# 10XGenomics/supernova

Measured on AMD Instinct MI355X. Metric: Gk-mers/s through count+graph at k=48, 1.2B×150bp; bit-exact counts, higher is better.
Workload: dtype u64

## Files before the change

supernova_amd/csrc/snk_graph.h:

```cpp
#pragma once
#include "snk_ctx.h"
#include "snk_kernels.h"

struct snk_graph_out {
    uint8_t* ctx;
    uint32_t* counts;
    unsigned long long* spectrum;
    uint32_t spectrum_bins;
    uint64_t n_unitigs;
    uint64_t total_bases;
    uint64_t* unitig_off;
    uint8_t* unitig_bases;
    uint32_t* unitig_group;
    uint32_t n_circles;
    uint32_t rank_rounds;
    uint64_t n_boundary;
    uint64_t n_fragments;
};

int snk_graph_sort(snk_ctx* ctx, hipStream_t st, uint32_t K, uint64_t n, snk_u128* keys_in, uint64_t* vals_in,
                   snk_u128* keys_out, uint64_t* vals_out, char* err, size_t errcap);
int snk_graph_build(snk_ctx* ctx, hipStream_t st, uint32_t K, const snk_u128* keys, const uint64_t* vals, uint64_t n,
                    uint32_t do_prune, bool want_unitigs, snk_graph_out* out, char* err, size_t errcap);

// ... 39 lines not shown
int snk_join_rank(snk_ctx* ctx, hipStream_t st, uint64_t F, const uint32_t* nk, uint32_t* flink, const uint2** rk_out, uint8_t** circ_out,
                  uint32_t* n_circles, uint32_t* rounds, char* err, size_t errcap, uint8_t* circ_given = nullptr);
int snk_join_place(snk_ctx* ctx, hipStream_t st, const uint2* rk, const uint32_t* nk, const uint8_t* circ, uint64_t f0, uint64_t Fl,
                   snk_placement* pl, char* err, size_t errcap, uint64_t rk_f0 = 0);
struct snk_prank {
    uint64_t ns, m, k0, k1, n_rec;
    const uint32_t* w;
    uint32_t* link;
    unsigned long long* wrec;
    uint32_t* spl_state;
    uint4* w1_share;
    uint4* rec;
};
int snk_prank_begin(snk_ctx* ctx, hipStream_t st, uint64_t F, const uint32_t* nk, uint32_t* link, uint32_t rank, uint32_t world, snk_prank* P, char* err,
                    size_t errcap);
int snk_prank_walk(snk_ctx* ctx, hipStream_t st, snk_prank* P, const uint4* w1_all, uint32_t* circles, uint32_t* rounds, char* err, size_t errcap,
                   uint8_t* circ = nullptr , uint32_t* n_cut = nullptr);
int snk_prank_route(snk_ctx* ctx, hipStream_t st, snk_prank* P, const unsigned long long* d_frag_off, uint32_t world,
                    unsigned long long* d_cursor , void* d_out, char* err, size_t errcap);
int snk_prank_apply(snk_ctx* ctx, hipStream_t st, const void* d_rec, uint64_t n, unsigned long long state_base, uint64_t n_local_states,
                    const uint2** rk_out, char* err, size_t errcap);
int snk_join_emit(snk_ctx* ctx, hipStream_t st, uint32_t K, uint64_t F, const uint32_t* nk, const uint32_t* gfid, const uint32_t* pl_pid,
                  const unsigned long long* pl_koff, const unsigned long long* pl_N, const uint8_t* pl_circ, uint32_t pid_base, uint64_t n_pid,
                  const uint64_t* boff, const uint8_t* fbases, const uint32_t* fgroup, snk_join_out* out, char* err, size_t errcap);
int snk_dist_answer(snk_ctx* ctx, hipStream_t st, snk_dist_graph* g, const void* d_queries, uint64_t nq, void* d_ans, char* err,
                    size_t errcap);
int snk_dist_apply(snk_ctx* ctx, hipStream_t st, snk_dist_graph* g, const void* d_qbuf, const void* d_ans, uint64_t nq,
                   const unsigned long long* d_qoff, char* err, size_t errcap);
int snk_dist_join(snk_ctx* ctx, hipStream_t st, uint32_t K, uint64_t F, const uint32_t* nk, const unsigned long long* hl_self,
                  const unsigned long long* hl_nb, const uint64_t* boff, const uint8_t* fbases, uint64_t total_fbases,
                  snk_join_out* out, char* err, size_t errcap, const uint32_t* fgroup = nullptr, const uint32_t* sfrag = nullptr,
                  uint64_t n_states = 0);
int snk_dist_links_query(snk_ctx* ctx, hipStream_t st, const snk_frag_out* fr, const unsigned long long* d_node_off, uint32_t world,
                         unsigned long long my_end_base, unsigned long long* d_cursor, void* d_qbuf, char* err, size_t errcap);
int snk_dist_links_answer(snk_ctx* ctx, hipStream_t st, const snk_frag_out* fr, const void* d_queries, uint64_t nq, unsigned long long my_state_base,
                          uint64_t n_local_states, unsigned long long my_end_base, void* d_ans, char* err, size_t errcap);
int snk_dist_links_apply_regions(snk_ctx* ctx, hipStream_t st, const snk_frag_out* fr, const void* d_qbuf, const void* d_ans, uint32_t world, uint64_t cap,
                                 const unsigned long long* counts, uint32_t** flink_out, char* err, size_t errcap);

struct snk_table;
struct snk_bl_state {
    const snk_table* tab;
    uint32_t K, rank, world, NB_total, NBl, do_prune, force_dist;
    uint4* desc;
    uint32_t nchunks, nbig;
    uint32_t* biglist;
    uint8_t *ctx, *pend, *premote;
    uint32_t *counts, *nbr, *rq;
    uint32_t* rq_idx;
    uint16_t* rq_meta;
    unsigned long long* index;
    uint64_t index_mask, n_boundary;
    unsigned long long *qcount, *qcursor;
    unsigned long long* spec;
    uint32_t want_spec, spec_over;
// ... 11 lines not shown
```

supernova_amd/csrc/snk_graph.hip:

```cpp
#include <string.h>
#include <cstring>
#include <rocprim/rocprim.hpp>

#include "snk_ctx.h"
#include "snk_common.h"
#include "snk_kernels.h"
#include "snk_graph.h"
#include "snk_stages.h"

namespace {

constexpr uint32_t NONE = 0xFFFFFFFFu;
constexpr int TB = 256;

__device__ __forceinline__ snk_kmer load_key(const snk_u128* keys, uint64_t i) {
    const uint64_t* p = reinterpret_cast<const uint64_t*>(keys + i);
    snk_kmer k;
    k.lo = p[0];
    k.hi = p[1];
    return k;
}

__global__ void __launch_bounds__(TB) index_build_kernel(const snk_u128* __restrict__ keys, uint64_t n,
                                                         unsigned long long* __restrict__ tab, uint64_t mask) {
// ... 1066 lines not shown
__device__ __forceinline__ uint32_t ld_u32_any(const uint8_t* p) { return reinterpret_cast<const u32_any*>(p)->v; }
__device__ __forceinline__ void st_u32_any(uint8_t* p, uint32_t v) { reinterpret_cast<u32_any*>(p)->v = v; }
__device__ __forceinline__ void copy16(uint8_t* dst, const uint8_t* src, bool rev) {
    if (!rev) {
        const uint32_t a = ld_u32_any(src), b = ld_u32_any(src + 4), c = ld_u32_any(src + 8), d = ld_u32_any(src + 12);
        st_u32_any(dst, a); st_u32_any(dst + 4, b); st_u32_any(dst + 8, c); st_u32_any(dst + 12, d);
    } else {
        const uint32_t a = ld_u32_any(src - 4), b = ld_u32_any(src - 8), c = ld_u32_any(src - 12), d = ld_u32_any(src - 16);
        st_u32_any(dst, __builtin_bswap32(a) ^ 0x03030303u); st_u32_any(dst + 4, __builtin_bswap32(b) ^ 0x03030303u);
        st_u32_any(dst + 8, __builtin_bswap32(c) ^ 0x03030303u); st_u32_any(dst + 12, __builtin_bswap32(d) ^ 0x03030303u);
    }
}
constexpr uint32_t JCH = 4096;
__global__ void __launch_bounds__(TB) jchunks_kernel(const uint64_t* __restrict__ boff, uint64_t F, uint32_t* __restrict__ nch) {
    uint64_t f = (uint64_t)blockIdx.x * TB + threadIdx.x;
    if (f >= F) return;
    nch[f] = (uint32_t)((boff[f + 1] - boff[f] + JCH - 1) / JCH);
}
__global__ void __launch_bounds__(TB) jchunk_owner_kernel(const uint32_t* __restrict__ choff, uint64_t F, uint32_t* __restrict__ owner) {
    uint64_t f = (uint64_t)blockIdx.x * TB + threadIdx.x;
    if (f >= F) return;
    if (choff[f + 1] > choff[f]) owner[choff[f]] = (uint32_t)f;
}
__global__ void __launch_bounds__(256) jemit_kernel(uint64_t F, const uint64_t* __restrict__ boff, const uint8_t* __restrict__ fbases,
                                                    const uint32_t* __restrict__ pl_pid, const unsigned long long* __restrict__ pl_koff,
                                                    const uint32_t* __restrict__ nk, const uint64_t* __restrict__ poff, uint32_t pid_base,
                                                    uint32_t K, uint8_t* __restrict__ prov) {
    for (uint64_t f = (uint64_t)blockIdx.x * 32 + (threadIdx.x >> 3); f < F; f += (uint64_t)gridDim.x * 32) {
    const uint32_t sub = threadIdx.x & 7u;
    const unsigned long long ko = pl_koff[f];
    const bool rc = (ko & PL_RC) != 0;
    const uint32_t skip = (ko & ~PL_RC) == 0 ? 0u : K - 1;
    const uint32_t len = nk[f] + K - 1 - skip;
    const uint8_t* src = fbases + boff[f] + (rc ? 0u : skip);
    uint8_t* dst = prov + poff[pl_pid[f] - pid_base] + (ko & ~PL_RC) + skip;
    uint32_t head = (4u - (uint32_t)((uintptr_t)dst & 3u)) & 3u;
    if (head > len) head = len;
    if (sub < head) dst[sub] = rc ? (uint8_t)(src[len - 1 - sub] ^ 3u) : src[sub];
    const uint32_t ndw = (len - head) >> 2;
    for (uint32_t j = sub; j < ndw; j += 8) {
        const uint32_t o = head + 4 * j;
        const uint32_t v = rc ? (__builtin_bswap32(ld_u32_any(src + len - 4 - o)) ^ 0x03030303u) : ld_u32_any(src + o);
        *reinterpret_cast<uint32_t*>(dst + o) = v;
    }
    const uint32_t t0 = head + 4 * ndw;
    if (sub < len - t0) { const uint32_t q = t0 + sub; dst[q] = rc ? (uint8_t)(src[len - 1 - q] ^ 3u) : src[q]; }
    }
}
__global__ void __launch_bounds__(TB) jform_kernel(const uint64_t* __restrict__ uoff, uint64_t U, const uint8_t* __restrict__ prov,
                                                   uint8_t* __restrict__ urev) {
    uint64_t u = (uint64_t)blockIdx.x * TB + threadIdx.x;
    if (u >= U) return;
    const uint8_t* b = prov + uoff[u];
    uint64_t len = uoff[u + 1] - uoff[u];
    uint8_t rev = 0;
    if (len & 1) rev = (b[len / 2] & 2) ? 1 : 0;
    else {
        for (uint64_t i = 0, j = len; i < j; ++i) {
            uint8_t f = b[i], r = (uint8_t)(b[--j] ^ 3);
            if (f < r) break;
            if (r < f) { rev = 1; break; }
        }
    }
    urev[u] = rev;
}
__global__ void __launch_bounds__(TB) jfinal_kernel(const uint64_t* __restrict__ uoff, const uint32_t* __restrict__ uowner_of_chunk,
                                                    const uint32_t* __restrict__ uchoff, const uint8_t* __restrict__ urev,
                                                    const uint8_t* __restrict__ prov, uint8_t* __restrict__ out) {
    const uint32_t item = blockIdx.x;
// ... 144 lines not shown
        void* tmp;
        if ((rc = snk_ctx_alloc(ctx, tb, &tmp, err, errcap))) return rc;
        SNK_HIP_TRY(rocprim::inclusive_scan(tmp, tb, owner, owner, (size_t)total, rocprim::maximum<uint32_t>(), st));
    }
    *choff_out = choff;
    *owner_out = owner;
    *total_out = total;
    return SNK_OK;
}

int snk_dist_answer(snk_ctx* ctx, hipStream_t st, snk_dist_graph* g, const void* d_queries, uint64_t nq, void* d_ans, char* err,
                    size_t errcap) {
    SNK_HIP_TRY(snk_launch(answer_kernel, snk_blocks(nq, TB), TB, 0, st, (const unsigned long long*)d_queries, nq, g->keys, g->index, g->index_mask, (uint32_t*)d_ans));
    return SNK_OK;
}
int snk_dist_apply(snk_ctx* ctx, hipStream_t st, snk_dist_graph* g, const void* d_qbuf, const void* d_ans, uint64_t nq,
                   const unsigned long long* d_qoff, char* err, size_t errcap) {
    SNK_HIP_TRY(snk_launch(apply_answers_kernel, snk_blocks(nq, TB), TB, 0, st, (const unsigned long long*)d_qbuf, (const uint32_t*)d_ans, nq, d_qoff, g->world, g->do_prune, reinterpret_cast<uint32_t*>(g->ctx), g->rq_idx, g->rq_meta));
    return SNK_OK;
}

int snk_dist_join(snk_ctx* ctx, hipStream_t st, uint32_t K, uint64_t F, const uint32_t* nk, const unsigned long long* hl_self,
                  const unsigned long long* hl_nb, const uint64_t* boff, const uint8_t* fbases, uint64_t total_fbases,
                  snk_join_out* out, char* err, size_t errcap, const uint32_t* fgroup, const uint32_t* sfrag, uint64_t n_states) {
    memset(out, 0, sizeof *out);
    if (F == 0) return snk_join_emit(ctx, st, K, 0, nullptr, nullptr, nullptr, nullptr, nullptr, nullptr, 0, 0, nullptr, nullptr, nullptr, out, err, errcap);
    if (F >= (1ull << 31)) return snk_fail(SNK_E_UNSUPPORTED, err, errcap, "more than 2^31 fragments at the join (%llu)", (unsigned long long)F);
    const uint64_t ne = 2 * F;
    uint32_t* flink;
    G_ALLOC(flink, uint32_t, ne);
    if (sfrag) {
        SNK_HIP_TRY(snk_launch(jmatch_direct_kernel, snk_blocks(ne, TB), TB, 0, st, hl_self, hl_nb, ne, sfrag, n_states, flink));
    } else {
        uint64_t tg = 1024;
        while (tg < 2 * ne) tg <<= 1;
        unsigned long long* hk;
        uint32_t* hv;
        G_ALLOC(hk, unsigned long long, tg);
        G_ALLOC(hv, uint32_t, tg);
        SNK_HIP_TRY(hipMemsetAsync(hk, 0, tg * 8, st));
        SNK_HIP_TRY(snk_launch(jhash_build_kernel, snk_blocks(ne, TB), TB, 0, st, hl_self, ne, hk, hv, tg - 1));
        SNK_HIP_TRY(snk_launch(jmatch_kernel, snk_blocks(ne, TB), TB, 0, st, hl_self, hl_nb, ne, hk, hv, tg - 1, flink));
    }
    uint8_t* circ;
    G_ALLOC(circ, uint8_t, ne + 1);
    SNK_HIP_TRY(hipMemsetAsync(circ, 0, ne + 1, st));
    const uint2* rk;
    int rc = rank_lists(ctx, st, flink, F, nk, circ, &rk, &out->n_circles, &out->rank_rounds, err, errcap);
    if (rc) return rc;
    snk_placement pl;
    if ((rc = snk_join_place(ctx, st, rk, nk, circ, 0, F, &pl, err, errcap))) return rc;
    const uint32_t nc = out->n_circles, rr = out->rank_rounds;
    if ((rc = snk_join_emit(ctx, st, K, F, nk, nullptr, pl.pid, pl.koff, pl.N, pl.circ, 0, ne, boff, fbases, fgroup, out, err, errcap))) return rc;
    out->n_circles = nc;
    out->rank_rounds = rr;
    return SNK_OK;
}

int snk_join_rank(snk_ctx* ctx, hipStream_t st, uint64_t F, const uint32_t* nk, uint32_t* flink, const uint2** rk_out, uint8_t** circ_out,
                  uint32_t* n_circles, uint32_t* rounds, char* err, size_t errcap, uint8_t* circ_given) {
    if (F >= (1ull << 31)) return snk_fail(SNK_E_UNSUPPORTED, err, errcap, "more than 2^31 fragments at the join (%llu)", (unsigned long long)F);
    uint8_t* circ = circ_given;
    if (!circ) {
        G_ALLOC(circ, uint8_t, 2 * F + 1);
        SNK_HIP_TRY(hipMemsetAsync(circ, 0, 2 * F + 1, st));
    }
    *circ_out = circ;
    *n_circles = 0;
    *rounds = 0;
    if (F == 0) { *rk_out = nullptr; return SNK_OK; }
    return rank_lists(ctx, st, flink, F, nk, circ, rk_out, n_circles, rounds, err, errcap);
}

int snk_join_place(snk_ctx* ctx, hipStream_t st, const uint2* rk, const uint32_t* nk, const uint8_t* circ, uint64_t f0, uint64_t Fl,
                   snk_placement* pl, char* err, size_t errcap, uint64_t rk_f0) {
    memset(pl, 0, sizeof *pl);
// ... 4 lines not shown
    SNK_HIP_TRY(snk_launch(jplace_kernel, snk_blocks(Fl, TB), TB, 0, st, rk, rk_f0, nk, circ, f0, Fl, pl->pid, pl->koff, pl->N, pl->circ));
    return SNK_OK;
}

__global__ void __launch_bounds__(256) jdbg_count_kernel(const uint8_t* __restrict__ b, uint64_t n, unsigned long long* __restrict__ out) {
    unsigned long long c = 0;
    for (uint64_t i = (uint64_t)blockIdx.x * 256 + threadIdx.x; i < n; i += (uint64_t)gridDim.x * 256) c += b[i] > 3 ? 1ull : 0ull;
    if (c) atomicAdd(out, c);
}
static int jdbg_count(snk_ctx* ctx, hipStream_t st, const char* what, const uint8_t* b, uint64_t n, char* err, size_t errcap) {
    unsigned long long* d;
    G_ALLOC(d, unsigned long long, 1);
    SNK_HIP_TRY(hipMemsetAsync(d, 0, 8, st));
    SNK_HIP_TRY(snk_launch(jdbg_count_kernel, 4096, 256, 0, st, b, n, d));
    unsigned long long h = 0;
    SNK_HIP_TRY(hipMemcpyAsync(&h, d, 8, hipMemcpyDeviceToHost, st));
    SNK_HIP_TRY(snk_sync(st));
    fprintf(stderr, "[snk join dbg] %s: %llu of %llu bytes are not bases\n", what, h, (unsigned long long)n);
    return SNK_OK;
}

int snk_join_emit(snk_ctx* ctx, hipStream_t st, uint32_t K, uint64_t F, const uint32_t* nk, const uint32_t* gfid, const uint32_t* pl_pid,
                  const unsigned long long* pl_koff, const unsigned long long* pl_N, const uint8_t* pl_circ, uint32_t pid_base, uint64_t n_pid,
                  const uint64_t* boff, const uint8_t* fbases, const uint32_t* fgroup, snk_join_out* out, char* err, size_t errcap) {
    memset(out, 0, sizeof *out);
    if (F == 0) {
        G_ALLOC(out->unitig_off, uint64_t, 1);
        SNK_HIP_TRY(hipMemsetAsync(out->unitig_off, 0, 8, st));
        return SNK_OK;
    }
    int rc;
    uint32_t *hflag, *hidx;
    uint64_t *hlen, *hoff;
    G_ALLOC(hflag, uint32_t, F + 1);
    G_ALLOC(hidx, uint32_t, F + 1);
    G_ALLOC(hlen, uint64_t, F + 1);
    G_ALLOC(hoff, uint64_t, F + 1);
    SNK_HIP_TRY(hipMemsetAsync(hflag + F, 0, 4, st));
    SNK_HIP_TRY(hipMemsetAsync(hlen + F, 0, 8, st));
    SNK_HIP_TRY(snk_launch(jhead_kernel, snk_blocks(F, TB), TB, 0, st, pl_pid, pl_koff, pl_N, gfid, F, K, hflag, hlen));
    if ((rc = excl_scan<uint32_t>(ctx, st, hflag, hidx, F + 1, err, errcap))) return rc;
    if ((rc = excl_scan<uint64_t>(ctx, st, hlen, hoff, F + 1, err, errcap))) return rc;
    uint32_t h_nu = 0;
    uint64_t h_tot = 0;
    SNK_HIP_TRY(hipMemcpyAsync(&h_nu, hidx + F, 4, hipMemcpyDeviceToHost, st));
    SNK_HIP_TRY(hipMemcpyAsync(&h_tot, hoff + F, 8, hipMemcpyDeviceToHost, st));
    SNK_HIP_TRY(snk_sync(st));
    const uint64_t U = h_nu;
    const uint64_t chunks_ub = U ? h_tot / JCH + U : 0;
    uint64_t *poff, *uoff;
    uint8_t *ucirc, *prov, *final_bases, *urev;
    G_ALLOC(poff, uint64_t, n_pid + 1);
    G_ALLOC(uoff, uint64_t, U + 1);
    G_ALLOC(ucirc, uint8_t, U + 1);
    G_ALLOC(urev, uint8_t, U + 1);
    uint32_t* ugroup = nullptr;
    if (fgroup) G_ALLOC(ugroup, uint32_t, U + 1);
    G_ALLOC(prov, uint8_t, h_tot + 1);
    G_ALLOC(final_bases, uint8_t, h_tot + 1);
    const bool jdbg = snk_opt_u32(ctx, SNK_OPT_join_dbg) != 0;
    if (jdbg) { SNK_HIP_TRY(hipMemsetAsync(prov, 0xEE, h_tot + 1, st)); SNK_HIP_TRY(hipMemsetAsync(final_bases, 0xEE, h_tot + 1, st)); fprintf(stderr, "[snk join dbg] F %llu unitigs %llu bases %llu\n", (unsigned long long)F, (unsigned long long)U, (unsigned long long)h_tot); }
    SNK_HIP_TRY(snk_launch(jhead_place_kernel, snk_blocks(F, TB), TB, 0, st, pl_pid, pl_circ, hflag, hidx, hoff, F, pid_base, poff, uoff, ucirc, fgroup, ugroup));
    SNK_HIP_TRY(hipMemcpyAsync(uoff + U, hoff + F, 8, hipMemcpyDeviceToDevice, st));
    SNK_HIP_TRY(snk_launch(jemit_kernel, snk_blocks_capped(F, 32, 1ull << std::min(22u, snk_opt_u32(ctx, SNK_OPT_emit_grid_log2))), 256, 0, st, F, boff, fbases, pl_pid, pl_koff, nk, poff, pid_base, K, prov));
    if (jdbg && (rc = jdbg_count(ctx, st, "provisional bases after the fragments' copies", prov, h_tot, err, errcap))) return rc;
    {
        uint32_t *clist, *ccnt;
        G_ALLOC(clist, uint32_t, U + 1);
        G_ALLOC(ccnt, uint32_t, 4);
        SNK_HIP_TRY(hipMemsetAsync(ccnt, 0, 4, st));
        SNK_HIP_TRY(snk_launch(jcirc_list_kernel, snk_blocks(U, TB), TB, 0, st, ucirc, U, clist, ccnt));
        const uint64_t cg = U < 1024 ? U : 1024;
        if (K == 48) SNK_HIP_TRY(snk_launch(jcircle_kernel<48>, cg, 256, 0, st, clist, ccnt, uoff, prov, final_bases));
        else SNK_HIP_TRY(snk_launch(jcircle_kernel<60>, cg, 256, 0, st, clist, ccnt, uoff, prov, final_bases));
    }
    SNK_HIP_TRY(snk_launch(jform_kernel, snk_blocks(U, TB), TB, 0, st, uoff, U, prov, urev));
    uint32_t *unch, *uchoff, *uowner, utotal = 0;
    G_ALLOC(unch, uint32_t, U + 1);
    SNK_HIP_TRY(hipMemsetAsync(unch + U, 0, 4, st));
    SNK_HIP_TRY(snk_launch(jchunks_kernel, snk_blocks(U, TB), TB, 0, st, uoff, U, unch));
    if ((rc = chunk_owners(ctx, st, unch, U, &uchoff, &uowner, &utotal, err, errcap, chunks_ub))) return rc;
    SNK_HIP_TRY(snk_launch(jfinal_kernel, utotal, 256, 0, st, uoff, uowner, uchoff, urev, prov, final_bases));
    if (jdbg && (rc = jdbg_count(ctx, st, "oriented bases", final_bases, h_tot, err, errcap))) return rc;
    uint64_t* noff = uoff;
    uint8_t* obases = final_bases;
    uint8_t* ocirc = ucirc;
    uint32_t* ogroup = ugroup;
// ... 226 lines not shown
```

supernova_amd/csrc/snk_local.hip:

```cpp
#include <string.h>
#include <cstring>
#include <rocprim/rocprim.hpp>

#include <type_traits>

#include "snk_ctx.h"
#include "snk_common.h"
#include "snk_kernels.h"
#include "snk_graph.h"
#include "snk_stages.h"

namespace {

constexpr uint32_t NONE = 0xFFFFFFFFu;
constexpr unsigned long long NONE64 = ~0ull;
constexpr uint16_t NONE16 = 0xFFFFu;
constexpr int TB = 256;

struct chunk_src {
    const uint32_t* chunk_n;
    const uint32_t* chunk_base;
    const uint4* extra;
    const unsigned long long* region_off;
    uint32_t NB, n_extra, n_regions;
// ... 449 lines not shown
};
template <int K, int CAP, int T, bool BIG, bool EMIT, bool DIST, bool GR>
__global__ void __launch_bounds__(T) bl_frag_kernel(const uint4* __restrict__ desc, const uint32_t* __restrict__ biglist_in,
                                                    const snk_u128* __restrict__ keys, const uint8_t* __restrict__ ctx,
                                                    const uint8_t* __restrict__ pend, const uint32_t* __restrict__ nbr,
                                                    const uint32_t* __restrict__ rq, bl_dist_args da, uint32_t* __restrict__ nfrag,
                                                    const uint32_t* __restrict__ foff, const uint64_t* __restrict__ boff,
                                                    uint32_t* __restrict__ nk, unsigned long long* __restrict__ hl_self,
                                                    unsigned long long* __restrict__ hl_nb, uint64_t* __restrict__ bstart,
                                                    uint8_t* __restrict__ fbases, uint32_t* __restrict__ fgroup, uint32_t* __restrict__ sfrag, bl_extra_pool xp) {
    constexpr int SPT = (2 * CAP + T - 1) / T;
    constexpr int NPT = (CAP + T - 1) / T;
    constexpr bool ONEW = T == 64;
    typedef typename std::conditional<(K <= 48 && !GR), uint32_t, uint64_t>::type klo_w;
    constexpr int KLS = (K <= 48 && !GR) ? 32 : 0;
    __shared__ uint64_t khi[ONEW ? 1 : CAP];
    __shared__ klo_w klo[ONEW ? 1 : CAP];
    __shared__ uint16_t nbL[2 * CAP];
    typedef typename std::conditional<(CAP <= 256), uint32_t, uint64_t>::type wrec_t;
    constexpr int FB = CAP <= 256 ? 10 : 16;
    constexpr uint32_t FM = (1u << FB) - 1u;
    __shared__ uint16_t lnk[2 * CAP];
    __shared__ wrec_t wr[2 * CAP];
    constexpr bool WIDE = (uint32_t)CAP * (uint32_t)K > 65535u;
    uint16_t* foffL = nbL;
    __shared__ uint32_t frel[WIDE ? CAP : 1];
    __shared__ uint16_t hnode[CAP];
    __shared__ uint8_t ctxL[CAP], pendL[CAP];
    __shared__ uint32_t fcnt, bcnt, changed;
    const int tid = threadIdx.x;
    const uint32_t c = BIG ? biglist_in[blockIdx.x] : blockIdx.x;
    const chunk_t ch = chunk_get(desc, c);
    if (ch.n == 0) return;
    if (!BIG && ch.n > (uint32_t)CAP) return;
    const uint32_t n = ch.n;
    const uint32_t c_foff = EMIT ? foff[c] : 0u;
    const uint64_t c_boff = EMIT ? boff[c] : 0ull;
    if constexpr (!ONEW) {
        if (tid == 0) { fcnt = 0; bcnt = 0; changed = 0; }
    }
    uint32_t w_frags = 0, w_bases = 0;
    snk_kmer kq[NPT] = {};
    {
        uint32_t cq[NPT], pq[NPT];
        uint32_t nq[NPT];
#pragma unroll
        for (int q = 0; q < NPT; ++q) {
            const uint32_t i = tid + q * T;
            if (i < n) {
                const uint64_t gi = ch.base + i;
                if (EMIT) kq[q] = load_key(keys, gi);
                cq[q] = ctx[gi];
                pq[q] = pend[gi];
                nq[q] = nbr[gi];
            }
        }
#pragma unroll
        for (int q = 0; q < NPT; ++q) {
            const uint32_t i = tid + q * T;
            if (i < n) {
// ... 125 lines not shown
            const uint32_t a = da.rq_idx[2 * gi + side];
            if (a == NONE) return NONE64;
            const uint32_t meta = da.rq_meta[2 * gi + side];
            const uint32_t fs = side ^ 1u ^ (meta >> 15);
            return 2ull * (da.node_off[meta & 0x7FFFu] + a) + fs;
        }
        const uint32_t a = rq[2 * gi + side];
        if (a == NONE) return NONE64;
        const uint32_t rev = a & 1u, fs = side ^ 1u ^ rev;
        return 2ull * ((DIST ? da.my_node_off : 0ull) + (a >> 1)) + fs;
    };
    auto describe = [&](uint32_t lf, uint32_t rel, uint32_t pid, uint32_t other, uint32_t cnt, uint32_t head_node, bool head_rc, uint32_t group) {
        const uint64_t f = (uint64_t)c_foff + lf;
        nk[f] = cnt;
        hl_self[2 * f] = 2ull * ((DIST ? da.my_node_off : 0ull) + ch.base) + pid;
        hl_self[2 * f + 1] = 2ull * ((DIST ? da.my_node_off : 0ull) + ch.base) + other;
        hl_nb[2 * f] = half_link(pid);
        hl_nb[2 * f + 1] = half_link(other);
        bstart[f] = c_boff + rel;
        if (sfrag) { sfrag[2 * ch.base + pid] = (uint32_t)(2 * f); sfrag[2 * ch.base + other] = (uint32_t)(2 * f + 1); }
        if (GR) fgroup[f] = group;
        if constexpr (WIDE) { foffL[pid] = (uint16_t)lf; frel[lf] = rel; }
        else foffL[pid] = (uint16_t)rel;
        hnode[lf] = (uint16_t)((head_node << 1) | (head_rc ? 1u : 0u));
    };

#pragma unroll
    for (int q = 0; q < NPT; ++q) {
        if ((uint32_t)(q * T) >= n) break;
        const uint32_t i = tid + q * T;
        bool head = false, fwd = false;
        uint32_t tR = 0, tL = 0, cnt = 0;
        if (i < n && w_next(2 * i) == FM) {
            tR = w_tail(2 * i); tL = w_tail(2 * i + 1);
            const uint32_t dR = w_dist(2 * i), dL = w_dist(2 * i + 1);
            fwd = tL < tR;
            head = (fwd ? dL : dR) == 0;
            cnt = dR + dL + 1u;
        }
        const uint32_t nb = head ? cnt + (uint32_t)K - 1u : 0u;
        uint32_t lf = 0, rel = 0;
        if constexpr (ONEW) {
            const unsigned long long hm = __ballot(head);
            if (hm == 0) continue;
            const uint32_t incl = snk_wave_scan_incl(nb);
            lf = w_frags + (uint32_t)__popcll(hm & ((1ull << tid) - 1ull));
            rel = w_bases + incl - nb;
            w_frags += (uint32_t)__popcll(hm);
            w_bases += (uint32_t)__builtin_amdgcn_readlane((int)incl, 63);
        } else if (head) {
            lf = atomicAdd(&fcnt, 1u);
            rel = atomicAdd(&bcnt, nb);
        }
        if (head) describe(lf, rel, fwd ? tL : tR, fwd ? tR : tL, cnt, i, !fwd, GR ? (uint32_t)own_key(q, i).lo : 0u);
    }
    for (uint32_t i = tid; i < n; i += T) {
        if (w_next(2 * i) == FM) continue;
        uint32_t cur = i << 1, cnt = 1;
        const snk_kmer ki = key_of(i);
        bool closed = false;
        while (cnt <= n) {
            const uint32_t l = lnk[cur];
            if (l == NONE16) break;
            const uint32_t j = l >> 1;
            if (j == i) { closed = true; break; }
            if (snk_kmer_lt(key_of(j), ki)) break;
            cur = l ^ 1u;
            ++cnt;
        }
        if (closed) {
            const unsigned long long xf = atomicAdd(&xp.cur[0], 1ull);
            const unsigned long long xb = atomicAdd(&xp.cur[1], (unsigned long long)(cnt + K - 1));
            if (xf < xp.fcap && xb + cnt + K - 1 <= xp.bcap) {
                uint32_t e = i << 1;
                for (uint32_t q = 1; q < cnt; ++q) e = lnk[e] ^ 1u;
                const uint64_t f = xp.f0 + xf, bo = xp.b0 + xb;
                const uint32_t pid = (i << 1) | 1u;
                nk[f] = cnt;
                hl_self[2 * f] = 2ull * ((DIST ? da.my_node_off : 0ull) + ch.base) + pid;
                hl_self[2 * f + 1] = 2ull * ((DIST ? da.my_node_off : 0ull) + ch.base) + e;
                hl_nb[2 * f] = NONE64;
                hl_nb[2 * f + 1] = NONE64;
                bstart[f] = bo;
                if (sfrag) { sfrag[2 * ch.base + pid] = (uint32_t)(2 * f); sfrag[2 * ch.base + e] = (uint32_t)(2 * f + 1); }
                if (GR) fgroup[f] = (uint32_t)ki.lo;
                snk_kmer k = ki;
                for (int b = 0; b < K; ++b) fbases[bo + b] = (uint8_t)oriented_base<K>(k, false, b);
                uint32_t curs = i << 1;
                for (uint32_t pos = 1; pos < cnt; ++pos) {
                    const uint32_t l = lnk[curs];
                    k = key_of(l >> 1);
                    fbases[bo + (K - 1) + pos] = (uint8_t)oriented_base<K>(k, (l & 1u) == 0, K - 1);
                    curs = l ^ 1u;
                }
            }
        }
    }
    __syncthreads();
#pragma unroll
    for (int q = 0; q < NPT; ++q) {
        const uint32_t i = tid + q * T;
        if (i >= n || w_next(2 * i) != FM) continue;
        const uint32_t tR = w_tail(2 * i), tL = w_tail(2 * i + 1), dR = w_dist(2 * i), dL = w_dist(2 * i + 1);
        const bool fwd = tL < tR;
        const uint32_t pos = fwd ? dL : dR;
        if (pos == 0) continue;
        const snk_kmer k = own_key(q, i);
        uint32_t fo = foffL[fwd ? tL : tR];
        if constexpr (WIDE) fo = frel[fo];
        fbases[c_boff + fo + (K - 1) + pos] = (uint8_t)oriented_base<K>(k, !fwd, K - 1);
    }
    struct __attribute__((packed)) u32_any { uint32_t v; };
    uint32_t nheads = w_frags;
    if constexpr (!ONEW) nheads = fcnt;
    constexpr int HPI = T / 16;
    static_assert(K % 4 == 0 && K / 4 <= 16, "a head is K / 4 dwords, one per lane of its group");
    for (uint32_t h0 = 0; h0 < nheads; h0 += HPI) {
        const uint32_t h = h0 + (tid >> 4);
        const int q = tid & 15;
        const bool act = h < nheads && q < K / 4;
        const uint32_t hn = act ? hnode[h] : 0u;
        const uint32_t i = hn >> 1;
        const bool rc = hn & 1u;
        snk_kmer k;
        if constexpr (ONEW) {
            k.hi = 0; k.lo = 0;
#pragma unroll
            for (int s = 0; s < NPT; ++s) {
                if ((uint32_t)(s * T) >= n) break;
                const int src = (int)(i & 63u);
                const uint32_t a0 = (uint32_t)__shfl((int)(uint32_t)(kq[s].hi >> 32), src), a1 = (uint32_t)__shfl((int)(uint32_t)kq[s].hi, src);
                const uint32_t a2 = (uint32_t)__shfl((int)(uint32_t)(kq[s].lo >> 32), src);
                uint32_t a3 = 0;
                if constexpr (K > 48) a3 = (uint32_t)__shfl((int)(uint32_t)kq[s].lo, src);
                if ((i >> 6) == (uint32_t)s) { k.hi = ((uint64_t)a0 << 32) | a1; k.lo = ((uint64_t)a2 << 32) | a3; }
            }
        } else {
            k = key_of(i);
        }
        if (act) {
            uint32_t fo;
            if constexpr (WIDE) fo = frel[h];
            else { const uint32_t tR = w_tail(2 * i), tL = w_tail(2 * i + 1); fo = foffL[tL < tR ? tL : tR]; }
            const uint32_t v = oriented_base<K>(k, rc, 4 * q) | (oriented_base<K>(k, rc, 4 * q + 1) << 8) | (oriented_base<K>(k, rc, 4 * q + 2) << 16) |
                               (oriented_base<K>(k, rc, 4 * q + 3) << 24);
            reinterpret_cast<u32_any*>(fbases + c_boff + fo + 4 * q)->v = v;
        }
    }
}

__global__ void __launch_bounds__(TB) bl_chunk_bases_kernel(const uint4* __restrict__ desc, const uint32_t* __restrict__ nfrag, uint32_t nchunks,
                                                            uint32_t K, uint64_t* __restrict__ nbases) {
    const uint32_t c = blockIdx.x * TB + threadIdx.x;
    if (c > nchunks) return;
    if (c == nchunks) { nbases[c] = 0; return; }
    const uint32_t n = desc[c].y;
    nbases[c] = nfrag[c] ? (uint64_t)n + (uint64_t)(K - 1) * nfrag[c] : 0ull;
}

__global__ void __launch_bounds__(TB) bl_pack_vals_kernel(const uint32_t* __restrict__ counts, const uint8_t* __restrict__ ctx,
                                                          uint64_t n, uint64_t* __restrict__ vals) {
    const uint64_t i = (uint64_t)blockIdx.x * TB + threadIdx.x;
    if (i < n) vals[i] = ((uint64_t)counts[i] << 8) | ctx[i];
}
__global__ void __launch_bounds__(TB) bl_unpack_vals_kernel(const uint64_t* __restrict__ vals, uint64_t n,
                                                            uint32_t* __restrict__ counts, uint8_t* __restrict__ ctx) {
    const uint64_t i = (uint64_t)blockIdx.x * TB + threadIdx.x;
    if (i < n) { counts[i] = (uint32_t)(vals[i] >> 8); ctx[i] = (uint8_t)(vals[i] & 0xFFu); }
}

// ... 198 lines not shown
    while (tg < 2 * h_bnd) tg <<= 1;
    const bool fused_ok = index0 && !h_gaveup && h_bnd * 4 <= tg0 * 3;
    if (fused_ok) { B->index = index0; tg = tg0; }
    else {
        if (index0) snk_ctx_release_block(ctx, index0);
        G_ALLOC(B->index, unsigned long long, tg);
        SNK_HIP_TRY(hipMemsetAsync(B->index, 0, tg * 8, st));
    }
    B->index_mask = tg - 1;
    if (h_bnd) {
        if (!fused_ok) SNK_HIP_TRY(snk_launch(bl_index_build_kernel, snk_blocks(n, TB), TB, 0, st, tab->keys, B->pend, n, B->index, tg - 1));
        SNK_HIP_TRY(snk_launch(bl_resolve_kernel<K, GR>, snk_blocks(n, 8 * TB), TB, 0, st, tab->keys, B->pend, n,
                               B->index, tg - 1, B->do_prune, B->ctx, B->rq, (const uint8_t*)B->premote));
    }
    return SNK_OK;
}

template <int K, bool DIST, bool GR>
static int bl_fragments_impl(snk_ctx* ctx, hipStream_t st, snk_bl_state* B, const bl_dist_args& da, snk_frag_out* out, char* err,
                             size_t errcap) {
    const snk_table* tab = B->tab;
    const uint32_t nchunks = B->nchunks, h_nbig = B->nbig;
    uint32_t *nfrag, *foff;
    uint64_t *nbases, *boff;
    G_ALLOC(nfrag, uint32_t, (uint64_t)nchunks + 1);
    G_ALLOC(foff, uint32_t, (uint64_t)nchunks + 1);
    G_ALLOC(nbases, uint64_t, (uint64_t)nchunks + 1);
    G_ALLOC(boff, uint64_t, (uint64_t)nchunks + 1);
    SNK_HIP_TRY(hipMemsetAsync(nfrag, 0, ((uint64_t)nchunks + 1) * 4, st));
    bl_extra_pool xp0;
    memset(&xp0, 0, sizeof xp0);
    SNK_HIP_TRY(snk_launch(bl_frag_kernel<K, SCAP, ST, false, false, DIST, GR>, nchunks, ST, 0, st, (const uint4*)B->desc,
                           (const uint32_t*)nullptr, tab->keys, B->ctx, B->pend, B->nbr, B->rq, da, nfrag, (const uint32_t*)nullptr,
                           (const uint64_t*)nullptr, (uint32_t*)nullptr, (unsigned long long*)nullptr, (unsigned long long*)nullptr,
                           (uint64_t*)nullptr, (uint8_t*)nullptr, (uint32_t*)nullptr, (uint32_t*)nullptr, xp0));
    SNK_HIP_TRY(snk_launch(bl_frag_kernel<K, BCAP, BT, true, false, DIST, GR>, h_nbig, BT, 0, st, (const uint4*)B->desc,
                           (const uint32_t*)B->biglist, tab->keys, B->ctx, B->pend, B->nbr, B->rq, da, nfrag, (const uint32_t*)nullptr,
                           (const uint64_t*)nullptr, (uint32_t*)nullptr, (unsigned long long*)nullptr, (unsigned long long*)nullptr,
                           (uint64_t*)nullptr, (uint8_t*)nullptr, (uint32_t*)nullptr, (uint32_t*)nullptr, xp0));
    SNK_HIP_TRY(snk_launch(bl_chunk_bases_kernel, snk_blocks((uint64_t)nchunks + 1, TB), TB, 0, st, (const uint4*)B->desc, nfrag, nchunks,
                           (uint32_t)K, nbases));
    int rc;
    if ((rc = excl_scan<uint32_t>(ctx, st, nfrag, foff, (size_t)nchunks + 1, err, errcap))) return rc;
    if ((rc = excl_scan<uint64_t>(ctx, st, nbases, boff, (size_t)nchunks + 1, err, errcap))) return rc;
    uint32_t h_F = 0;
    uint64_t h_B = 0;
    SNK_HIP_TRY(hipMemcpyAsync(&h_F, foff + nchunks, 4, hipMemcpyDeviceToHost, st));
    SNK_HIP_TRY(hipMemcpyAsync(&h_B, boff + nchunks, 8, hipMemcpyDeviceToHost, st));
    SNK_HIP_TRY(snk_sync(st));
    unsigned long long* xcur;
    G_ALLOC(xcur, unsigned long long, 2);
    const uint32_t pool0 = snk_opt_u32(ctx, SNK_OPT_bl_pool);
    uint64_t xf_cap = pool0 ? pool0 + h_F / 256 : 0, xb_cap = xf_cap * (K + 63);
    unsigned long long h_x[2] = {0, 0};
    for (int attempt = 0; attempt < 2; ++attempt) {
        ctx->last_bl_attempts = (uint32_t)attempt + 1;
        G_ALLOC(out->nk, uint32_t, (uint64_t)h_F + xf_cap + 1);
        G_ALLOC(out->hl_self, unsigned long long, 2ull * (h_F + xf_cap) + 2);
        G_ALLOC(out->hl_nb, unsigned long long, 2ull * (h_F + xf_cap) + 2);
        G_ALLOC(out->boff, uint64_t, (uint64_t)h_F + xf_cap + 2);
        G_ALLOC(out->bases, uint8_t, h_B + xb_cap + 16);
        out->fgroup = nullptr;
        if (GR) G_ALLOC(out->fgroup, uint32_t, (uint64_t)h_F + xf_cap + 1);
        G_ALLOC(out->sfrag, uint32_t, 2 * tab->n + 2);
        SNK_HIP_TRY(hipMemsetAsync(xcur, 0, 16, st));
        bl_extra_pool xp;
        xp.cur = xcur;
        xp.f0 = h_F;
        xp.b0 = h_B;
        xp.fcap = xf_cap;
        xp.bcap = xb_cap;
// ... 43 lines not shown
        return snk_fail(SNK_E_INTERNAL, err, errcap, "bucket-local graph: chunk capacity %d is below the count table's limit", BCAP);
    snk_phase_timer tm(st);
    tm.mark();
    snk_bl_state B;
    memset(&B, 0, sizeof B);
    B.tab = tab;
    B.K = K;
    B.world = 1;
    B.do_prune = do_prune;
    B.want_spec = sort_table ? 0u : 1u;
    int rc = bl_prune_impl<K, GR>(ctx, st, &B, err, errcap);
    if (rc) return rc;
    tm.mark();
    tm.mark();
    out->n_boundary = B.n_boundary;
    if (want_unitigs) {
        snk_frag_out fo;
        memset(&fo, 0, sizeof fo);
        bl_dist_args da;
        memset(&da, 0, sizeof da);
        if ((rc = bl_fragments_impl<K, false, GR>(ctx, st, &B, da, &fo, err, errcap))) return rc;
        tm.mark();
        snk_join_out jo;
        rc = snk_dist_join(ctx, st, K, fo.n_frags, fo.nk, fo.hl_self, fo.hl_nb, fo.boff, fo.bases, fo.total_bases, &jo, err, errcap, fo.fgroup, fo.sfrag, 2 * n);
        if (rc) return rc;
        tm.mark();
        out->n_unitigs = jo.n_unitigs;
        out->total_bases = jo.total_bases;
        out->unitig_off = jo.unitig_off;
        out->unitig_bases = jo.unitig_bases;
        out->unitig_group = jo.unitig_group;
        out->n_circles = jo.n_circles;
        out->rank_rounds = jo.rank_rounds;
        out->n_fragments = fo.n_frags;
    } else {
        G_ALLOC(out->unitig_off, uint64_t, 2);
        SNK_HIP_TRY(hipMemsetAsync(out->unitig_off, 0, 16, st));
        G_ALLOC(out->unitig_bases, uint8_t, 16);
        tm.mark();
        tm.mark();
    }
    out->ctx = B.ctx;
    out->counts = B.counts;
    if (sort_table) {
        uint64_t *v_in, *v_out;
        snk_u128* k_out;
        G_ALLOC(v_in, uint64_t, n + 1);
// ... 91 lines not shown
```

Baseline: 102.0.

## Skip storing head k-mer bases in local fragments; rebuild them from keys at emit

In the non-distributed local path, fragments no longer store the K-1 leading bases of their head k-mer. Each fragment's base region is sized to its k-mer count, so the per-chunk base-count kernel and its scan are dropped. The join emit kernel gains a HEADS variant that rebuilds those leading bases from the head key in the table (reverse-complementing when needed, masking group bits) and shuffles it across the 8-lane subgroup. This cuts fragment-base writes and memory, at the cost of more index arithmetic and an extra key load in the emit kernel.

```diff
diff --git a/supernova_amd/csrc/snk_graph.h b/supernova_amd/csrc/snk_graph.h
--- a/supernova_amd/csrc/snk_graph.h
+++ b/supernova_amd/csrc/snk_graph.h
@@ -85,7 +85,8 @@
                     const uint2** rk_out, char* err, size_t errcap);
 int snk_join_emit(snk_ctx* ctx, hipStream_t st, uint32_t K, uint64_t F, const uint32_t* nk, const uint32_t* gfid, const uint32_t* pl_pid,
                   const unsigned long long* pl_koff, const unsigned long long* pl_N, const uint8_t* pl_circ, uint32_t pid_base, uint64_t n_pid,
-                  const uint64_t* boff, const uint8_t* fbases, const uint32_t* fgroup, snk_join_out* out, char* err, size_t errcap);
+                  const uint64_t* boff, const uint8_t* fbases, const uint32_t* fgroup, snk_join_out* out, char* err, size_t errcap,
+                  const snk_u128* head_keys = nullptr, const unsigned long long* hl_self = nullptr, uint64_t key_lo_mask = ~0ull);
 int snk_dist_answer(snk_ctx* ctx, hipStream_t st, snk_dist_graph* g, const void* d_queries, uint64_t nq, void* d_ans, char* err,
                     size_t errcap);
 int snk_dist_apply(snk_ctx* ctx, hipStream_t st, snk_dist_graph* g, const void* d_qbuf, const void* d_ans, uint64_t nq,
@@ -93,7 +94,7 @@
 int snk_dist_join(snk_ctx* ctx, hipStream_t st, uint32_t K, uint64_t F, const uint32_t* nk, const unsigned long long* hl_self,
                   const unsigned long long* hl_nb, const uint64_t* boff, const uint8_t* fbases, uint64_t total_fbases,
                   snk_join_out* out, char* err, size_t errcap, const uint32_t* fgroup = nullptr, const uint32_t* sfrag = nullptr,
-                  uint64_t n_states = 0);
+                  uint64_t n_states = 0, const snk_u128* head_keys = nullptr, uint64_t key_lo_mask = ~0ull);
 int snk_dist_links_query(snk_ctx* ctx, hipStream_t st, const snk_frag_out* fr, const unsigned long long* d_node_off, uint32_t world,
                          unsigned long long my_end_base, unsigned long long* d_cursor, void* d_qbuf, char* err, size_t errcap);
 int snk_dist_links_answer(snk_ctx* ctx, hipStream_t st, const snk_frag_out* fr, const void* d_queries, uint64_t nq, unsigned long long my_state_base,
diff --git a/supernova_amd/csrc/snk_graph.hip b/supernova_amd/csrc/snk_graph.hip
--- a/supernova_amd/csrc/snk_graph.hip
+++ b/supernova_amd/csrc/snk_graph.hip
@@ -1112,29 +1112,81 @@
     if (f >= F) return;
     if (choff[f + 1] > choff[f]) owner[choff[f]] = (uint32_t)f;
 }
+__device__ __forceinline__ snk_kmer jemit_rc(snk_kmer k, uint32_t K) {
+    const uint64_t a = snk_rev2(~k.lo), b = snk_rev2(~k.hi);
+    const uint32_t S = 128u - 2u * K;
+    snk_kmer r;
+    r.hi = (a << S) | (b >> (64u - S));
+    r.lo = b << S;
+    return r;
+}
+__device__ __forceinline__ uint32_t jemit_key4(snk_kmer k, uint32_t p0) {
+    const uint32_t sh = 2u * p0;
+    const uint64_t top = sh == 0 ? k.hi : sh < 64u ? ((k.hi << sh) | (k.lo >> (64u - sh))) : (k.lo << (sh - 64u));
+    const uint32_t b8 = (uint32_t)(top >> 56);
+    return (b8 >> 6) | (((b8 >> 4) & 3u) << 8) | (((b8 >> 2) & 3u) << 16) | ((b8 & 3u) << 24);
+}
+template <bool HEADS>
 __global__ void __launch_bounds__(256) jemit_kernel(uint64_t F, const uint64_t* __restrict__ boff, const uint8_t* __restrict__ fbases,
                                                     const uint32_t* __restrict__ pl_pid, const unsigned long long* __restrict__ pl_koff,
                                                     const uint32_t* __restrict__ nk, const uint64_t* __restrict__ poff, uint32_t pid_base,
-                                                    uint32_t K, uint8_t* __restrict__ prov) {
+                                                    uint32_t K, uint8_t* __restrict__ prov, const snk_u128* __restrict__ keys,
+                                                    const unsigned long long* __restrict__ hl_self, uint64_t key_lo_mask) {
     for (uint64_t f = (uint64_t)blockIdx.x * 32 + (threadIdx.x >> 3); f < F; f += (uint64_t)gridDim.x * 32) {
     const uint32_t sub = threadIdx.x & 7u;
+    unsigned long long hs = 0;
+    if constexpr (HEADS) { if (sub == 0) hs = hl_self[2 * f]; }
     const unsigned long long ko = pl_koff[f];
     const bool rc = (ko & PL_RC) != 0;
     const uint32_t skip = (ko & ~PL_RC) == 0 ? 0u : K - 1;
     const uint32_t len = nk[f] + K - 1 - skip;
-    const uint8_t* src = fbases + boff[f] + (rc ? 0u : skip);
     uint8_t* dst = prov + poff[pl_pid[f] - pid_base] + (ko & ~PL_RC) + skip;
     uint32_t head = (4u - (uint32_t)((uintptr_t)dst & 3u)) & 3u;
     if (head > len) head = len;
-    if (sub < head) dst[sub] = rc ? (uint8_t)(src[len - 1 - sub] ^ 3u) : src[sub];
     const uint32_t ndw = (len - head) >> 2;
-    for (uint32_t j = sub; j < ndw; j += 8) {
-        const uint32_t o = head + 4 * j;
-        const uint32_t v = rc ? (__builtin_bswap32(ld_u32_any(src + len - 4 - o)) ^ 0x03030303u) : ld_u32_any(src + o);
-        *reinterpret_cast<uint32_t*>(dst + o) = v;
-    }
     const uint32_t t0 = head + 4 * ndw;
-    if (sub < len - t0) { const uint32_t q = t0 + sub; dst[q] = rc ? (uint8_t)(src[len - 1 - q] ^ 3u) : src[q]; }
+    if constexpr (!HEADS) {
+        const uint8_t* src = fbases + boff[f] + (rc ? 0u : skip);
+        if (sub < head) dst[sub] = rc ? (uint8_t)(src[len - 1 - sub] ^ 3u) : src[sub];
+        for (uint32_t j = sub; j < ndw; j += 8) {
+            const uint32_t o = head + 4 * j;
+            const uint32_t v = rc ? (__builtin_bswap32(ld_u32_any(src + len - 4 - o)) ^ 0x03030303u) : ld_u32_any(src + o);
+            *reinterpret_cast<uint32_t*>(dst + o) = v;
+        }
+        if (sub < len - t0) { const uint32_t q = t0 + sub; dst[q] = rc ? (uint8_t)(src[len - 1 - q] ^ 3u) : src[q]; }
+    } else {
+        const uint8_t* L = fbases + boff[f];
+        const uint32_t K1 = K - 1;
+        uint32_t w0 = 0, w1 = 0, w2 = 0, w3 = 0;
+        if ((rc || skip == 0) && sub == 0) {
+            snk_kmer k = load_key(keys, hs >> 1);
+            k.lo &= key_lo_mask;
+            if (!(hs & 1ull)) k = jemit_rc(k, K);
+            w0 = (uint32_t)(k.hi >> 32); w1 = (uint32_t)k.hi; w2 = (uint32_t)(k.lo >> 32); w3 = (uint32_t)k.lo;
+        }
+        w0 = (uint32_t)__shfl((int)w0, 0, 8); w1 = (uint32_t)__shfl((int)w1, 0, 8);
+        w2 = (uint32_t)__shfl((int)w2, 0, 8); w3 = (uint32_t)__shfl((int)w3, 0, 8);
+        snk_kmer hk;
+        hk.hi = ((uint64_t)w0 << 32) | w1;
+        hk.lo = ((uint64_t)w2 << 32) | w3;
+        auto S1 = [&](uint32_t p) -> uint32_t { return p < K1 ? (jemit_key4(hk, p) & 3u) : (uint32_t)L[p - K1]; };
+        auto S4 = [&](uint32_t p0) -> uint32_t {
+            if (p0 >= K1) return ld_u32_any(L + (p0 - K1));
+            uint32_t v = jemit_key4(hk, p0);
+            if (p0 + 3 >= K1) {
+                for (uint32_t b = 0; b < 4; ++b)
+                    if (p0 + b >= K1) v = (v & ~(0xFFu << (8 * b))) | ((uint32_t)L[p0 + b - K1] << (8 * b));
+            }
+            return v;
+        };
+        if (sub < head) dst[sub] = (uint8_t)(rc ? (S1(len - 1 - sub) ^ 3u) : S1(skip + sub));
+        for (uint32_t j = sub; j < ndw; j += 8) {
+            const uint32_t o = head + 4 * j;
+            const uint32_t v = rc ? (__builtin_bswap32(S4(len - 4 - o)) ^ 0x03030303u) : S4(skip + o);
+            *reinterpret_cast<uint32_t*>(dst + o) = v;
+        }
+        if (sub < len - t0) { const uint32_t q = t0 + sub; dst[q] = (uint8_t)(rc ? (S1(len - 1 - q) ^ 3u) : S1(skip + q)); }
+    }
     }
 }
 __global__ void __launch_bounds__(TB) jform_kernel(const uint64_t* __restrict__ uoff, uint64_t U, const uint8_t* __restrict__ prov,
@@ -1325,7 +1377,8 @@
 
 int snk_dist_join(snk_ctx* ctx, hipStream_t st, uint32_t K, uint64_t F, const uint32_t* nk, const unsigned long long* hl_self,
                   const unsigned long long* hl_nb, const uint64_t* boff, const uint8_t* fbases, uint64_t total_fbases,
-                  snk_join_out* out, char* err, size_t errcap, const uint32_t* fgroup, const uint32_t* sfrag, uint64_t n_states) {
+                  snk_join_out* out, char* err, size_t errcap, const uint32_t* fgroup, const uint32_t* sfrag, uint64_t n_states,
+                  const snk_u128* head_keys, uint64_t key_lo_mask) {
     memset(out, 0, sizeof *out);
     if (F == 0) return snk_join_emit(ctx, st, K, 0, nullptr, nullptr, nullptr, nullptr, nullptr, nullptr, 0, 0, nullptr, nullptr, nullptr, out, err, errcap);
     if (F >= (1ull << 31)) return snk_fail(SNK_E_UNSUPPORTED, err, errcap, "more than 2^31 fragments at the join (%llu)", (unsigned long long)F);
@@ -1354,7 +1407,7 @@
     snk_placement pl;
     if ((rc = snk_join_place(ctx, st, rk, nk, circ, 0, F, &pl, err, errcap))) return rc;
     const uint32_t nc = out->n_circles, rr = out->rank_rounds;
-    if ((rc = snk_join_emit(ctx, st, K, F, nk, nullptr, pl.pid, pl.koff, pl.N, pl.circ, 0, ne, boff, fbases, fgroup, out, err, errcap))) return rc;
+    if ((rc = snk_join_emit(ctx, st, K, F, nk, nullptr, pl.pid, pl.koff, pl.N, pl.circ, 0, ne, boff, fbases, fgroup, out, err, errcap, head_keys, hl_self, key_lo_mask))) return rc;
     out->n_circles = nc;
     out->rank_rounds = rr;
     return SNK_OK;
@@ -1405,7 +1458,8 @@
 
 int snk_join_emit(snk_ctx* ctx, hipStream_t st, uint32_t K, uint64_t F, const uint32_t* nk, const uint32_t* gfid, const uint32_t* pl_pid,
                   const unsigned long long* pl_koff, const unsigned long long* pl_N, const uint8_t* pl_circ, uint32_t pid_base, uint64_t n_pid,
-                  const uint64_t* boff, const uint8_t* fbases, const uint32_t* fgroup, snk_join_out* out, char* err, size_t errcap) {
+                  const uint64_t* boff, const uint8_t* fbases, const uint32_t* fgroup, snk_join_out* out, char* err, size_t errcap,
+                  const snk_u128* head_keys, const unsigned long long* hl_self, uint64_t key_lo_mask) {
     memset(out, 0, sizeof *out);
     if (F == 0) {
         G_ALLOC(out->unitig_off, uint64_t, 1);
@@ -1445,7 +1499,11 @@
     if (jdbg) { SNK_HIP_TRY(hipMemsetAsync(prov, 0xEE, h_tot + 1, st)); SNK_HIP_TRY(hipMemsetAsync(final_bases, 0xEE, h_tot + 1, st)); fprintf(stderr, "[snk join dbg] F %llu unitigs %llu bases %llu\n", (unsigned long long)F, (unsigned long long)U, (unsigned long long)h_tot); }
     SNK_HIP_TRY(snk_launch(jhead_place_kernel, snk_blocks(F, TB), TB, 0, st, pl_pid, pl_circ, hflag, hidx, hoff, F, pid_base, poff, uoff, ucirc, fgroup, ugroup));
     SNK_HIP_TRY(hipMemcpyAsync(uoff + U, hoff + F, 8, hipMemcpyDeviceToDevice, st));
-    SNK_HIP_TRY(snk_launch(jemit_kernel, snk_blocks_capped(F, 32, 1ull << std::min(22u, snk_opt_u32(ctx, SNK_OPT_emit_grid_log2))), 256, 0, st, F, boff, fbases, pl_pid, pl_koff, nk, poff, pid_base, K, prov));
+    {
+        const uint64_t eg = snk_blocks_capped(F, 32, 1ull << std::min(22u, snk_opt_u32(ctx, SNK_OPT_emit_grid_log2)));
+        if (head_keys) SNK_HIP_TRY(snk_launch(jemit_kernel<true>, eg, 256, 0, st, F, boff, fbases, pl_pid, pl_koff, nk, poff, pid_base, K, prov, head_keys, hl_self, key_lo_mask));
+        else SNK_HIP_TRY(snk_launch(jemit_kernel<false>, eg, 256, 0, st, F, boff, fbases, pl_pid, pl_koff, nk, poff, pid_base, K, prov, (const snk_u128*)nullptr, (const unsigned long long*)nullptr, ~0ull));
+    }
     if (jdbg && (rc = jdbg_count(ctx, st, "provisional bases after the fragments' copies", prov, h_tot, err, errcap))) return rc;
     {
         uint32_t *clist, *ccnt;
diff --git a/supernova_amd/csrc/snk_local.hip b/supernova_amd/csrc/snk_local.hip
--- a/supernova_amd/csrc/snk_local.hip
+++ b/supernova_amd/csrc/snk_local.hip
@@ -495,10 +495,10 @@
     constexpr uint32_t FM = (1u << FB) - 1u;
     __shared__ uint16_t lnk[2 * CAP];
     __shared__ wrec_t wr[2 * CAP];
-    constexpr bool WIDE = (uint32_t)CAP * (uint32_t)K > 65535u;
+    constexpr bool WIDE = DIST && (uint32_t)CAP * (uint32_t)K > 65535u;
     uint16_t* foffL = nbL;
     __shared__ uint32_t frel[WIDE ? CAP : 1];
-    __shared__ uint16_t hnode[CAP];
+    __shared__ uint16_t hnode[DIST ? CAP : 1];
     __shared__ uint8_t ctxL[CAP], pendL[CAP];
     __shared__ uint32_t fcnt, bcnt, changed;
     const int tid = threadIdx.x;
@@ -508,7 +508,7 @@
     if (!BIG && ch.n > (uint32_t)CAP) return;
     const uint32_t n = ch.n;
     const uint32_t c_foff = EMIT ? foff[c] : 0u;
-    const uint64_t c_boff = EMIT ? boff[c] : 0ull;
+    const uint64_t c_boff = DIST ? (EMIT ? boff[c] : 0ull) : ch.base;
     if constexpr (!ONEW) {
         if (tid == 0) { fcnt = 0; bcnt = 0; changed = 0; }
     }
@@ -680,7 +680,7 @@
         if (GR) fgroup[f] = group;
         if constexpr (WIDE) { foffL[pid] = (uint16_t)lf; frel[lf] = rel; }
         else foffL[pid] = (uint16_t)rel;
-        hnode[lf] = (uint16_t)((head_node << 1) | (head_rc ? 1u : 0u));
+        if constexpr (DIST) hnode[lf] = (uint16_t)((head_node << 1) | (head_rc ? 1u : 0u));
     };
 
 #pragma unroll
@@ -696,7 +696,7 @@
             head = (fwd ? dL : dR) == 0;
             cnt = dR + dL + 1u;
         }
-        const uint32_t nb = head ? cnt + (uint32_t)K - 1u : 0u;
+        const uint32_t nb = head ? cnt + (DIST ? (uint32_t)K - 1u : 0u) : 0u;
         uint32_t lf = 0, rel = 0;
         if constexpr (ONEW) {
             const unsigned long long hm = __ballot(head);
@@ -728,8 +728,9 @@
         }
         if (closed) {
             const unsigned long long xf = atomicAdd(&xp.cur[0], 1ull);
-            const unsigned long long xb = atomicAdd(&xp.cur[1], (unsigned long long)(cnt + K - 1));
-            if (xf < xp.fcap && xb + cnt + K - 1 <= xp.bcap) {
+            constexpr uint32_t HB = DIST ? K - 1 : 0;
+            const unsigned long long xb = atomicAdd(&xp.cur[1], (unsigned long long)(cnt + HB));
+            if (xf < xp.fcap && xb + cnt + HB <= xp.bcap) {
                 uint32_t e = i << 1;
                 for (uint32_t q = 1; q < cnt; ++q) e = lnk[e] ^ 1u;
                 const uint64_t f = xp.f0 + xf, bo = xp.b0 + xb;
@@ -743,12 +744,13 @@
                 if (sfrag) { sfrag[2 * ch.base + pid] = (uint32_t)(2 * f); sfrag[2 * ch.base + e] = (uint32_t)(2 * f + 1); }
                 if (GR) fgroup[f] = (uint32_t)ki.lo;
                 snk_kmer k = ki;
-                for (int b = 0; b < K; ++b) fbases[bo + b] = (uint8_t)oriented_base<K>(k, false, b);
+                if constexpr (DIST) { for (int b = 0; b < K; ++b) fbases[bo + b] = (uint8_t)oriented_base<K>(k, false, b); }
+                else fbases[bo] = (uint8_t)oriented_base<K>(k, false, K - 1);
                 uint32_t curs = i << 1;
                 for (uint32_t pos = 1; pos < cnt; ++pos) {
                     const uint32_t l = lnk[curs];
                     k = key_of(l >> 1);
-                    fbases[bo + (K - 1) + pos] = (uint8_t)oriented_base<K>(k, (l & 1u) == 0, K - 1);
+                    fbases[bo + HB + pos] = (uint8_t)oriented_base<K>(k, (l & 1u) == 0, K - 1);
                     curs = l ^ 1u;
                 }
             }
@@ -762,12 +764,13 @@
         const uint32_t tR = w_tail(2 * i), tL = w_tail(2 * i + 1), dR = w_dist(2 * i), dL = w_dist(2 * i + 1);
         const bool fwd = tL < tR;
         const uint32_t pos = fwd ? dL : dR;
-        if (pos == 0) continue;
+        if (DIST && pos == 0) continue;
         const snk_kmer k = own_key(q, i);
         uint32_t fo = foffL[fwd ? tL : tR];
         if constexpr (WIDE) fo = frel[fo];
-        fbases[c_boff + fo + (K - 1) + pos] = (uint8_t)oriented_base<K>(k, !fwd, K - 1);
-    }
+        fbases[c_boff + fo + (DIST ? K - 1 : 0) + pos] = (uint8_t)oriented_base<K>(k, !fwd, K - 1);
+    }
+    if constexpr (DIST) {
     struct __attribute__((packed)) u32_any { uint32_t v; };
     uint32_t nheads = w_frags;
     if constexpr (!ONEW) nheads = fcnt;
@@ -804,6 +807,7 @@
                                (oriented_base<K>(k, rc, 4 * q + 3) << 24);
             reinterpret_cast<u32_any*>(fbases + c_boff + fo + 4 * q)->v = v;
         }
+    }
     }
 }
 
@@ -1048,11 +1052,13 @@
     const snk_table* tab = B->tab;
     const uint32_t nchunks = B->nchunks, h_nbig = B->nbig;
     uint32_t *nfrag, *foff;
-    uint64_t *nbases, *boff;
+    uint64_t *nbases = nullptr, *boff = nullptr;
     G_ALLOC(nfrag, uint32_t, (uint64_t)nchunks + 1);
     G_ALLOC(foff, uint32_t, (uint64_t)nchunks + 1);
-    G_ALLOC(nbases, uint64_t, (uint64_t)nchunks + 1);
-    G_ALLOC(boff, uint64_t, (uint64_t)nchunks + 1);
+    if (DIST) {
+        G_ALLOC(nbases, uint64_t, (uint64_t)nchunks + 1);
+        G_ALLOC(boff, uint64_t, (uint64_t)nchunks + 1);
+    }
     SNK_HIP_TRY(hipMemsetAsync(nfrag, 0, ((uint64_t)nchunks + 1) * 4, st));
     bl_extra_pool xp0;
     memset(&xp0, 0, sizeof xp0);
@@ -1064,15 +1070,17 @@
                            (const uint32_t*)B->biglist, tab->keys, B->ctx, B->pend, B->nbr, B->rq, da, nfrag, (const uint32_t*)nullptr,
                            (const uint64_t*)nullptr, (uint32_t*)nullptr, (unsigned long long*)nullptr, (unsigned long long*)nullptr,
                            (uint64_t*)nullptr, (uint8_t*)nullptr, (uint32_t*)nullptr, (uint32_t*)nullptr, xp0));
-    SNK_HIP_TRY(snk_launch(bl_chunk_bases_kernel, snk_blocks((uint64_t)nchunks + 1, TB), TB, 0, st, (const uint4*)B->desc, nfrag, nchunks,
-                           (uint32_t)K, nbases));
     int rc;
     if ((rc = excl_scan<uint32_t>(ctx, st, nfrag, foff, (size_t)nchunks + 1, err, errcap))) return rc;
-    if ((rc = excl_scan<uint64_t>(ctx, st, nbases, boff, (size_t)nchunks + 1, err, errcap))) return rc;
     uint32_t h_F = 0;
-    uint64_t h_B = 0;
+    uint64_t h_B = tab->n;
+    if (DIST) {
+        SNK_HIP_TRY(snk_launch(bl_chunk_bases_kernel, snk_blocks((uint64_t)nchunks + 1, TB), TB, 0, st, (const uint4*)B->desc, nfrag, nchunks,
+                               (uint32_t)K, nbases));
+        if ((rc = excl_scan<uint64_t>(ctx, st, nbases, boff, (size_t)nchunks + 1, err, errcap))) return rc;
+        SNK_HIP_TRY(hipMemcpyAsync(&h_B, boff + nchunks, 8, hipMemcpyDeviceToHost, st));
+    }
     SNK_HIP_TRY(hipMemcpyAsync(&h_F, foff + nchunks, 4, hipMemcpyDeviceToHost, st));
-    SNK_HIP_TRY(hipMemcpyAsync(&h_B, boff + nchunks, 8, hipMemcpyDeviceToHost, st));
     SNK_HIP_TRY(snk_sync(st));
     unsigned long long* xcur;
     G_ALLOC(xcur, unsigned long long, 2);
@@ -1162,7 +1170,8 @@
         if ((rc = bl_fragments_impl<K, false, GR>(ctx, st, &B, da, &fo, err, errcap))) return rc;
         tm.mark();
         snk_join_out jo;
-        rc = snk_dist_join(ctx, st, K, fo.n_frags, fo.nk, fo.hl_self, fo.hl_nb, fo.boff, fo.bases, fo.total_bases, &jo, err, errcap, fo.fgroup, fo.sfrag, 2 * n);
+        rc = snk_dist_join(ctx, st, K, fo.n_frags, fo.nk, fo.hl_self, fo.hl_nb, fo.boff, fo.bases, fo.total_bases, &jo, err, errcap, fo.fgroup, fo.sfrag, 2 * n,
+                           tab->keys, GR ? ~0xFFFFFFFFull : ~0ull);
         if (rc) return rc;
         tm.mark();
         out->n_unitigs = jo.n_unitigs;
```

Result: no change. 102.7, median of 6 (+0.7%).
